# miuda-ai/lele

Hardware: AMD Instinct MI355X
Metric: STFT+mel GB/s (SenseVoice front-end: PCM -> log-mel -> LFR, algorithmic bytes); SenseVoiceSmall-shaped RTF in `sensevoice` (higher is better)
Workload: dtype f32

## Files before the change

### lele_amd/csrc/fe_core.h

```cpp
#pragma once
#include <stdint.h>

#if defined(__HIPCC__)
#define FE_HD __host__ __device__ __forceinline__
#else
#define FE_HD inline
#endif

namespace fe {

constexpr int kNfft = 512;
constexpr int kFrame = 400;
constexpr int kHop = 160;
constexpr int kBins = 257;
constexpr int kLanes = 16;
constexpr int kRegs = 32;
constexpr int kQ = 25;

FE_HD constexpr int rev4(int x) { return ((x & 1) << 3) | ((x & 2) << 1) | ((x & 4) >> 1) | ((x & 8) >> 3); }
FE_HD constexpr int rev5(int x) {
    return ((x & 1) << 4) | ((x & 2) << 2) | (x & 4) | ((x & 8) >> 2) | ((x & 16) >> 4);
}
FE_HD constexpr int tw_off(int s) { return (1 << (s - 1)) - 1; }

// ... 91 lines not shown
        if (rev5(r + 1) >= kQ) {
            s1[r] = x[r];
            s1[r + 1] = x[r];
        } else {
            s1[r] = fadd(x[r], x[r + 1]);
            s1[r + 1] = fsub(x[r], x[r + 1]);
        }
    }
    {
        const float wr = tw_re[tw_off(2) + 1], wi = tw_im[tw_off(2) + 1];
#pragma unroll
        for (int b = 0; b < kRegs; b += 4) {
            a[b] = cmk(fadd(s1[b], s1[b + 2]), 0.0f);
            a[b + 2] = cmk(fsub(s1[b], s1[b + 2]), 0.0f);
            const float tr = fmul(wr, s1[b + 3]);
            const float ti = fmul(wi, s1[b + 3]);
            a[b + 1] = cmk(fadd(s1[b + 1], tr), ti);
            a[b + 3] = cmk(fsub(s1[b + 1], tr), -ti);
        }
    }
#pragma unroll
    for (int b = 0; b < kRegs; b += 8) {
#pragma unroll
        for (int k = 0; k < 4; ++k) {
            const float wr = tw_re[tw_off(3) + k], wi = tw_im[tw_off(3) + k];
            if ((k & 1) == 0) {
                const float e = a[b + k].x, o = a[b + 4 + k].x;
                const float tr = fmul(wr, o);
                const float ti = fmul(wi, o);
                a[b + k] = cmk(fadd(e, tr), ti);
                a[b + 4 + k] = cmk(fsub(e, tr), -ti);
            } else {
                bfly_fma(make_tw(wr, wi), a[b + k], a[b + 4 + k]);
            }
        }
    }
#pragma unroll
    for (int s = 4; s <= 5; ++s) {
        const int half = 1 << (s - 1);
#pragma unroll
        for (int b = 0; b < kRegs; b += 2 * half) {
            {
                const cf e = a[b], o = a[b + half];
                a[b] = cadd(e, o);
                a[b + half] = csub(e, o);
            }
#pragma unroll
            for (int k = 1; k < half; ++k)
                bfly_fma(make_tw(tw_re[tw_off(s) + k], tw_im[tw_off(s) + k]), a[b + k], a[b + half + k]);
        }
    }
}

constexpr int kTwConstN = 31;
constexpr uint32_t kTwConstRe[kTwConstN] = {
    0x3f800000u, 0x3f800000u, 0xb33bbd2eu, 0x3f800000u, 0x3f3504f3u, 0xb33bbd2eu, 0xbf3504f3u, 0x3f800000u,
    0x3f6c835eu, 0x3f3504f3u, 0x3ec3ef15u, 0xb33bbd2eu, 0xbec3ef18u, 0xbf3504f3u, 0xbf6c8360u, 0x3f800000u,
    0x3f7b14beu, 0x3f6c835eu, 0x3f54db31u, 0x3f3504f3u, 0x3f0e39d9u, 0x3ec3ef15u, 0x3e47c5bcu, 0xb33bbd2eu,
    0xbe47c5c2u, 0xbec3ef18u, 0xbf0e39dcu, 0xbf3504f3u, 0xbf54db32u, 0xbf6c8360u, 0xbf7b14bfu};
constexpr uint32_t kTwConstIm[kTwConstN] = {
    0x80000000u, 0x80000000u, 0xbf800000u, 0x80000000u, 0xbf3504f3u, 0xbf800000u, 0xbf3504f3u, 0x80000000u,
    0xbec3ef16u, 0xbf3504f3u, 0xbf6c835eu, 0xbf800000u, 0xbf6c835eu, 0xbf3504f3u, 0xbec3ef10u, 0x80000000u,
    0xbe47c5c2u, 0xbec3ef16u, 0xbf0e39dau, 0xbf3504f3u, 0xbf54db32u, 0xbf6c835eu, 0xbf7b14bfu, 0xbf800000u,
    0xbf7b14beu, 0xbf6c835eu, 0xbf54db30u, 0xbf3504f3u, 0xbf0e39d9u, 0xbec3ef10u, 0xbe47c5c1u};
FE_HD bool tw_const_used(int i) {
    return i == tw_off(2) + 1 || (i >= tw_off(3) && i < tw_off(4)) || (i > tw_off(4) && i < tw_off(5)) ||
           (i > tw_off(5) && i < kTwConstN);
}
struct TwConst {
    bool im;
    FE_HD float operator[](int i) const { return __builtin_bit_cast(float, im ? kTwConstIm[i] : kTwConstRe[i]); }
};
inline bool tw_const_matches(const float* tw_re, const float* tw_im) {
    for (int i = 0; i < kTwConstN; ++i) {
        if (!tw_const_used(i)) continue;
        if (__builtin_bit_cast(uint32_t, tw_re[i]) != kTwConstRe[i] || __builtin_bit_cast(uint32_t, tw_im[i]) != kTwConstIm[i]) return false;
    }
    return true;
}

template <typename TWF>
FE_HD void phase_b(cf* b, int c, int rho, const TWF& twf, float* re256) {
#pragma unroll
    for (int s = 6; s <= 8; ++s) {
        const int hv = 1 << (s - 6);
#pragma unroll
        for (int k = 0; k < hv; ++k) {
            const cf w = twf(tw_off(s) + k * 32 + rho * 16 + c);
            const Tw tw = make_tw(w.x, w.y);
#pragma unroll
            for (int base = 0; base < 16; base += 2 * hv) bfly_fma(tw, b[base + k], b[base + hv + k]);
        }
    }
#pragma unroll
    for (int k = 0; k < 8; ++k) {
        const cf w = twf(tw_off(9) + k * 32 + rho * 16 + c);
        const cf t = tw_mul_fma(make_tw(w.x, w.y), b[8 + k]);
        if (k == 0) *re256 = fsub(b[0].x, t.x);
        b[k] = cadd(b[k], t);
    }
}


FE_HD float power(float re, float im) { return fadd(fmul(re, re), fmul(im, im)); }
FE_HD float power(cf z) {
    cf sq = cmulv(z, z);
// ... 12 lines not shown
```

### lele_amd/csrc/frontend.hip

```cpp
#include <type_traits>
#include "common.h"
#include "fe_core.h"

#include <math.h>

#include <algorithm>

using namespace lele;

namespace {

constexpr int kMaxMelRounds = 8;

struct FeDev {
    const float* tw_re;
    const float* tw_im;
    const float2* tw;
    const float* window;
    const float* melw;
    const float* melw_lds;
    const int* mel_start;
    const int* mel_step_off;
    int mel_rounds;
    int mel_steps;
    int n_mels;
    int lfr_m, lfr_n;
    int tile_dma;
};

struct GridBlock {
    __device__ __forceinline__ unsigned x() const { return blockIdx.x; }
    __device__ __forceinline__ unsigned y() const { return blockIdx.y; }
};
struct SegBlock {
    unsigned bx;
    __device__ __forceinline__ unsigned x() const { return bx; }
    __device__ __forceinline__ unsigned y() const { return 0u; }
};

struct FeSeg {
    int64_t start, len;
    int64_t num_frames, t_lfr;
    int64_t row0;
    int64_t block0;
};

constexpr int kSumRows = 66;
constexpr int kSumPitch = 164;

__global__ __launch_bounds__(64) void fe_frame_sum_kernel(const float* __restrict__ pcm, int64_t utt_stride,
                                                          int64_t pcm_len, int64_t num_frames,
                                                          float* __restrict__ mean_out, int aligned16) {
    __shared__ __attribute__((aligned(16))) float tile[kSumRows * kSumPitch];
    const int lane = threadIdx.x;
    const int64_t f0 = (int64_t)blockIdx.x * 64;
    const float* base = pcm + (int64_t)blockIdx.y * utt_stride;
    const int64_t s0 = f0 * fe::kHop;
    constexpr int kVecPerRow = fe::kHop / 4;
    constexpr int kVecs = kSumRows * kVecPerRow;
    constexpr int kIters = (kVecs + 63) / 64;
    constexpr int kBatch = 14;
    static_assert(kIters % kBatch == 0, "batching");
    for (int b0 = 0; b0 < kIters; b0 += kBatch) {
        float4 st[kBatch];
#pragma unroll
        for (int u = 0; u < kBatch; ++u) {
            const int idx = (b0 + u) * 64 + lane;
            int64_t s = s0 + 4 * (int64_t)idx;
            if (s + 3 >= pcm_len) s = aligned16 ? ((pcm_len - 4) & ~int64_t(3)) : (pcm_len - 4);
            if (s < 0) s = 0;
            const float* src = base + s;
            if (aligned16) {
                st[u] = *reinterpret_cast<const float4*>(src);
            } else {
                st[u] = make_float4(src[0], src[1], src[2], src[3]);
            }
        }
#pragma unroll
        for (int u = 0; u < kBatch; ++u) {
            const int idx = (b0 + u) * 64 + lane;
// ... 9 lines not shown
        }
    }
    __syncthreads();
    float sum = 0.0f;
#pragma unroll
    for (int seg = 0; seg < 3; ++seg) {
        const float* rowp = &tile[(lane + seg) * kSumPitch];
        const int nvec = seg < 2 ? kVecPerRow : (fe::kFrame - 2 * fe::kHop) / 4;
#pragma unroll 10
        for (int k = 0; k < nvec; ++k) {
            const float4 r = *reinterpret_cast<const float4*>(rowp + 4 * k);
            sum = sum + r.x;
            sum = sum + r.y;
            sum = sum + r.z;
            sum = sum + r.w;
        }
    }
    const int64_t f = f0 + lane;
    if (f < num_frames) mean_out[(int64_t)blockIdx.y * num_frames + f] = sum / (float)fe::kFrame;
}

constexpr int kFrameXchgFloats = 2 * 16 * fe::kXchgPitch;
constexpr int kWaveLdsFloats = 4 * kFrameXchgFloats;
constexpr int kPStride = 272;

struct TwLds {
    const float2* t;
    __device__ __forceinline__ float2 at(int i) const { return t[i]; }
};

__device__ __forceinline__ void fe_dma16(const void* gsrc, __attribute__((address_space(3))) char* lds_dst) {
    __builtin_amdgcn_global_load_lds((const __attribute__((address_space(1))) void*)gsrc, lds_dst, 16, 0, 0);
}

__device__ __forceinline__ const float* fe_const_table(const float* t, int pass) {
    auto c = (const __attribute__((address_space(4))) float*)t;
    asm("" : "+s"(c) : "s"(pass));
    return (const float*)c;
}

template <int MODE>
__device__ __forceinline__ float lane_rot_prev(float v, int p) {
    if (MODE == 1) {
        return __builtin_bit_cast(float,
                                  __builtin_amdgcn_update_dpp(0, __builtin_bit_cast(int, v), 0x121, 0xf, 0xf, true));
    } else {
        return __shfl(v, (p + 15) & 15, 16);
    }
}

constexpr int kStdMelLen[5] = {3, 4, 6, 10, 17};
constexpr int kStdMelOff[6] = {0, 3, 7, 13, 23, 40};

constexpr int kFeConstTw = 1, kFeLdsMel = 2, kFeLeanLds = 4;
typedef float fe_f2 __attribute__((ext_vector_type(2)));
typedef volatile __attribute__((address_space(3))) fe_f2* fe_lds_f2v;
__device__ __forceinline__ fe::cf fe_lds_read8(const float* p) {
    const fe_f2 t = *(fe_lds_f2v)p;
    return fe::cmk(t.x, t.y);
}
__device__ __forceinline__ void fe_lds_write8(float* p, fe::cf v) { *(fe_lds_f2v)p = (fe_f2){v.x, v.y}; }
constexpr int kMelLdsFloats = 768;
static_assert(fe::mel_lds_index(fe::kMelLdsWeights - 1, 15) < kMelLdsFloats && kStdMelOff[5] == fe::kMelLdsWeights, "the image holds the default bank");

template <int MODE, bool STDMEL, bool FUSED, int PASSES, bool LOWREG, int OPT, class Blk>
__device__ __forceinline__ void fe_main_body(const float* __restrict__ pcm, int64_t utt_stride,
                                             int64_t num_frames, int64_t t_lfr,
                                             const float* __restrict__ means, const FeDev& tb,
                                             float* __restrict__ out, float* __restrict__ logmel_out,
                                             int aligned16, float* s_melw, Blk bl) {
    constexpr int FR = 16 * PASSES;
    constexpr int kRows = FR + 2;
    constexpr int kXFloats = FUSED ? (kRows * kSumPitch > 4 * kWaveLdsFloats ? kRows * kSumPitch : 4 * kWaveLdsFloats)
                                   : 4 * kWaveLdsFloats;
    __shared__ float2 s_tw[LOWREG ? 480 : 512];
    __shared__ __attribute__((aligned(16))) float s_x[kXFloats];
    __shared__ float s_mean[64];
    __shared__ int s_mstart[16 * (STDMEL ? 5 : kMaxMelRounds)];
    __shared__ int s_moff[kMaxMelRounds + 1];
    constexpr int kTwBase = LOWREG ? 31 : 0;
    constexpr bool kConstTw = (OPT & kFeConstTw) != 0;
    constexpr bool kLdsMel = (OPT & kFeLdsMel) != 0;
    constexpr bool kLean = (OPT & kFeLeanLds) != 0;
    static_assert(!kLean || (kConstTw && kLdsMel), "the lean pass is a form of the constant-table kernel");
    static_assert(OPT == 0 || (STDMEL && FUSED && !LOWREG), "the constant / LDS table forms belong to the default bank's fused kernel");
    __shared__ __attribute__((aligned(16))) float s_melt[kLdsMel ? kMelLdsFloats : 4];
    static_assert(sizeof(s_tw) + sizeof(s_x) + sizeof(s_mean) + sizeof(s_mstart) + sizeof(s_moff) + sizeof(s_melt) <= 54613, "LDS of three workgroups fits a CU");

    const int lane = threadIdx.x & 63, wave = threadIdx.x >> 6;
    const int g = lane >> 4, p = lane & 15;
    constexpr int kVecPerRow = fe::kHop / 4;
    constexpr int kVecs = kRows * kVecPerRow;
    constexpr int kIters = (kVecs + 255) / 256;
    constexpr bool kTwDma = FUSED && !LOWREG;
    const bool tile_dma = FUSED && !LOWREG && aligned16 && tb.tile_dma;
    float4 st[FUSED ? kIters : 1];
    if constexpr (FUSED) {
        const float* run = pcm + (int64_t)bl.y() * utt_stride + (int64_t)bl.x() * FR * fe::kHop;
        const int64_t rem64 = utt_stride - (int64_t)bl.x() * FR * fe::kHop;
        const int rem = (int)(rem64 < (1 << 20) ? rem64 : (1 << 20));
        if (tile_dma) {
            constexpr int kSlotsPerRow = kSumPitch / 4;
            constexpr int kDma = (FR - 1 + 2) * kSlotsPerRow + (fe::kFrame - 2 * fe::kHop) / 4;
            constexpr int kDmaInstr = (kDma + 63) / 64;
            static_assert(kDmaInstr * 64 * 4 <= kXFloats, "the tile DMA stays inside s_x");
            auto* tile_lds = (__attribute__((address_space(3))) char*)s_x;
            static_assert(kSlotsPerRow == 41 && kDmaInstr * 64 * 1599 < (1 << 24), "i / 41 == (i * 1599) >> 16 for every slot");
            const unsigned last = 4u * (unsigned)rem - 16u;
            const int wave_s = __builtin_amdgcn_readfirstlane(wave);
#pragma unroll
            for (int u = 0; 4 * u < kDmaInstr; ++u) {
                const unsigned i = 256u * u + threadIdx.x;
                const unsigned ob = 16u * (i - ((i * 1599u) >> 16));
                if (4 * u + 3 < kDmaInstr || 4 * u + wave_s < kDmaInstr)
                    fe_dma16(reinterpret_cast<const char*>(run) + (ob < last ? ob : last), tile_lds + (4 * u + wave_s) * 1024);
            }
        }
        if (kTwDma && wave == 3) {
            auto* tw_lds = (__attribute__((address_space(3))) char*)s_tw;
#pragma unroll
            for (int k = 0; k < 4; ++k)
                fe_dma16(reinterpret_cast<const char*>(tb.tw) + 1024 * k + 16 * lane, tw_lds + 1024 * k);
        }
        if (kLdsMel && wave == 2) {
            auto* mel_lds = (__attribute__((address_space(3))) char*)s_melt;
#pragma unroll
            for (int k = 0; k < kMelLdsFloats / 256; ++k)
                fe_dma16(reinterpret_cast<const char*>(tb.melw_lds) + 1024 * k + 16 * lane, mel_lds + 1024 * k);
        }
        if (!tile_dma) {
#pragma unroll
            for (int u = 0; u < kIters; ++u) {
                const int idx = u * 256 + (int)threadIdx.x;
                int o = 4 * idx;
                if (o + 3 >= rem) o = aligned16 ? ((rem - 4) & ~3) : (rem - 4);
                const float* src = run + o;
                if (aligned16)
                    st[u] = *reinterpret_cast<const float4*>(src);
                else
                    st[u] = make_float4(src[0], src[1], src[2], src[3]);
            }
        }
    }
    if (!kTwDma)
        for (int i = threadIdx.x; i < 511 - kTwBase; i += 256) s_tw[i] = tb.tw[i + kTwBase];
    if (!STDMEL)
        for (int i = threadIdx.x; i < tb.mel_steps * 16; i += 256) s_melw[i] = tb.melw[i];
    if (threadIdx.x < tb.mel_rounds * 16) s_mstart[threadIdx.x] = tb.mel_start[threadIdx.x];
    if (threadIdx.x <= tb.mel_rounds) s_moff[threadIdx.x] = tb.mel_step_off[threadIdx.x];
    if (FUSED) {
        if (!tile_dma) {
#pragma unroll
            for (int u = 0; u < kIters; ++u) {
                const int idx = u * 256 + (int)threadIdx.x;
                if (idx < kVecs) {
                    const int row = idx / kVecPerRow, c = idx - row * kVecPerRow;
                    *reinterpret_cast<float4*>(&s_x[row * kSumPitch + 4 * c]) = st[u];
                }
            }
        }
        __builtin_amdgcn_s_waitcnt(0x0F70);
        __syncthreads();
    }
    const int h = fe::rev4(p);
    float* xw = s_x + wave * kWaveLdsFloats;
    float* xf = xw + g * kFrameXchgFloats;
    const float* base = pcm + (int64_t)bl.y() * utt_stride;
    const float* mean_u = means + (int64_t)bl.y() * num_frames;
    const int d_out = tb.n_mels * tb.lfr_m;
    float* out_u = out ? out + (int64_t)bl.y() * t_lfr * d_out : nullptr;
    float* lm_u = logmel_out ? logmel_out + (int64_t)bl.y() * num_frames * tb.n_mels : nullptr;

    float win[fe::kQ];
    if (!LOWREG) {
#pragma unroll
// ... 46 lines not shown
    const int f_first = (int)(bl.x() * FR) + wave * (4 * PASSES) + g;
    const int nfr = (int)num_frames, tl = (int)t_lfr;
    const int pad = (tb.lfr_m - 1) / 2;
    const unsigned blk_bytes = 4u * (unsigned)tb.n_mels, row_bytes = 4u * (unsigned)d_out;
    auto target_off = [&](int i, int b) { return (unsigned)i * row_bytes + (unsigned)b * blk_bytes + 4u * (unsigned)p; };
    int lfr_b = (f_first + pad) % tb.lfr_n, lfr_i = (f_first + pad) / tb.lfr_n;
    unsigned lfr_o = target_off(lfr_i, lfr_b);
    auto next_targets = [&]() {
        lfr_b += 4;
        if (tb.lfr_n >= 4) {
            const bool carry = lfr_b >= tb.lfr_n;
            lfr_b -= carry ? tb.lfr_n : 0;
            lfr_i += carry ? 1 : 0;
            lfr_o += carry ? 4u * blk_bytes + row_bytes - (unsigned)tb.lfr_n * blk_bytes : 4u * blk_bytes;
        } else {
            lfr_i += lfr_b / tb.lfr_n;
            lfr_b = lfr_b % tb.lfr_n;
            lfr_o = target_off(lfr_i, lfr_b);
        }
    };

    auto run_pass = [&](int pass, auto load_next_c) {
        constexpr bool load_next = decltype(load_next_c)::value;
        const int fi = f_first + pass * 4;
        const bool valid = fi < nfr;
        const float mean = FUSED ? s_mean[wave * (4 * PASSES) + pass * 4 + g] : mean_next;
        if (LOWREG) {
            int off = 0;
            asm volatile("" : "+v"(off));
#pragma unroll
            for (int q = 0; q < fe::kQ; ++q) win[q] = tb.window[p + 16 * q + off];
        }

        float v[fe::kQ];
        const float neg_mean = -mean;
#pragma unroll
        for (int q = 0; q < fe::kQ; ++q) v[q] = __builtin_fmaf(xr[q], 32768.0f, neg_mean);
        if (load_next) issue_loads(pass + 1);
        float xin[fe::kRegs];
#pragma unroll
        for (int r = 0; r < fe::kRegs; ++r) xin[r] = 0.0f;
        float k97;
        asm("v_mov_b32 %0, 0x3f7851ec" : "=v"(k97));
#pragma unroll
        for (int q = 0; q < fe::kQ; ++q) {
            const float send = (p == 15 && q > 0) ? v[q > 0 ? q - 1 : 0] : v[q];
            const float prev = lane_rot_prev<MODE>(send, p);
            float y = fe::fsub(v[q], fe::fmul(k97, prev));
            if (q == 0) y = (p == 0) ? v[0] : y;
            xin[fe::rev5(q)] = fe::fmul(y, win[q]);
        }

        fe::cf a[fe::kRegs];
        if constexpr (kConstTw)
            fe::phase_a_fast(xin, a, fe::TwConst{false}, fe::TwConst{true});
        else
            fe::phase_a_fast(xin, a, fe_const_table(tb.tw_re, pass), fe_const_table(tb.tw_im, pass));

        float pw[2][8];
        float p256 = 0.0f;
#pragma unroll
        for (int rho = 0; rho < 2; ++rho) {
            __builtin_amdgcn_wave_barrier();
#pragma unroll
            for (int cc = 0; cc < 16; ++cc) {
                const int slot = fe::xchg_slot(h, cc);
                if constexpr (kLean)
                    fe_lds_write8(xf + 2 * slot, a[rho * 16 + cc]);
                else
                    *reinterpret_cast<float2*>(xf + 2 * slot) = make_float2(a[rho * 16 + cc].x, a[rho * 16 + cc].y);
            }
            __builtin_amdgcn_wave_barrier();
            fe::cf bq[16];
#pragma unroll
            for (int vv = 0; vv < 16; ++vv) {
                if constexpr (kLean) {
                    bq[vv] = fe_lds_read8(xf + 2 * fe::xchg_slot(vv, p));
                } else {
                    const float2 t = *reinterpret_cast<const float2*>(xf + 2 * fe::xchg_slot(vv, p));
                    bq[vv] = fe::cmk(t.x, t.y);
                }
            }
            __builtin_amdgcn_wave_barrier();
            float re256 = 0.0f;
            fe::phase_b(bq, p, rho, [&](int i) { const float2 w = s_tw[i - kTwBase]; return fe::cmk(w.x, w.y); }, &re256);
            if (rho == 0) p256 = re256;
#pragma unroll
            for (int vv = 0; vv < 8; ++vv) {
                fe::cf z = bq[vv];
                if (vv == 0 && rho == 0) z = fe::cmk(z.x, (p == 0) ? 0.0f : z.y);
                pw[rho][vv] = fe::power(z);
            }
        }
        float* prow = xw + g * kPStride;
        __builtin_amdgcn_wave_barrier();
#pragma unroll
        for (int rho = 0; rho < 2; ++rho)
#pragma unroll
            for (int vv = 0; vv < 8; ++vv) prow[(2 * vv + rho) * 16 + p] = pw[rho][vv];
        if (p == 0) prow[256] = fe::power(p256, 0.0f);
        __builtin_amdgcn_wave_barrier();

        float vals[STDMEL ? 5 : kMaxMelRounds];
        float wl[kLdsMel ? fe::kMelLdsWeights : 1];
        if constexpr (kLdsMel) {
#pragma unroll
            for (int j = 0; j < fe::kMelLdsChunks; ++j) {
// ... 356 lines not shown
    const int per = n_mels / W;
    for (int v = lane; v < per * lfr_m; v += 64) {
        const int b = v / per, c = v - b * per;
        int64_t g = i * lfr_n + b - pad;
        g = g < 0 ? 0 : g;
        if (r.final) g = g > r.last_frame ? r.last_frame : g;
        LELE_DEV_ASSERT(g >= r.mel_base && g - r.mel_base < r.mel_carry + r.nf);
        const float* src = mel + (g - r.mel_base) * n_mels + W * c;
        float* d = dst + b * n_mels + W * c;
        if (VEC)
            __builtin_nontemporal_store(*reinterpret_cast<const fe_f4*>(src), reinterpret_cast<fe_f4*>(d));
        else
            __builtin_nontemporal_store(*src, d);
    }
}

__device__ __forceinline__ void fe_stream_move(float* region, int from, int count) {
    if (from == 0) return;
    for (int r0 = 0; r0 < count; r0 += 256 * kCompactRegs) {
        float v[kCompactRegs];
#pragma unroll
        for (int u = 0; u < kCompactRegs; ++u) {
            const int j = r0 + u * 256 + (int)threadIdx.x;
            v[u] = j < count ? region[from + j] : 0.0f;
        }
        __syncthreads();
#pragma unroll
        for (int u = 0; u < kCompactRegs; ++u) {
            const int j = r0 + u * 256 + (int)threadIdx.x;
            if (j < count) region[j] = v[u];
        }
    }
}
__global__ __launch_bounds__(256) void fe_stream_compact_kernel(const FeStreamRec* __restrict__ recs, float* pcm_state, int64_t pcm_pitch,
                                                                float* mel_state, int64_t mel_pitch, int n_mels) {
    const FeStreamRec r = recs[blockIdx.x];
    LELE_DEV_ASSERT(r.pcm_from + r.pcm_keep <= pcm_pitch && (int64_t)(r.mel_from + r.mel_keep) * n_mels <= mel_pitch);
    fe_stream_move(pcm_state + (int64_t)blockIdx.x * pcm_pitch, r.pcm_from, r.pcm_keep);
    fe_stream_move(mel_state + (int64_t)blockIdx.x * mel_pitch, r.mel_from * n_mels, r.mel_keep * n_mels);
}

}

struct LeleFrontend {
    LeleCtx* ctx = nullptr;
    LeleFeatureConfig cfg{};
    int64_t frame_len = 0, hop_len = 0, n_fft = 0;
    bool fast = false;
    bool std_mel = false;
    int dpp_mode = 0;
    bool fused = true;
    int opt = 0;
    bool lean = false;
    const float* g_window = nullptr;
    const int* g_mstart = nullptr;
    const int* g_moff = nullptr;
    const float* g_mw = nullptr;
    FeDev dev{};
    std::vector<void*> allocs;
    DevTables seg_tables;
    bool profiling = false;
    std::vector<hipEvent_t> events;
    size_t events_used = 0;
};

namespace {

static const float PI_F = 3.14159265358979323846264338327950288f;

void host_hann(int64_t size, std::vector<float>& w) {
    w.resize(size);
    if (size == 1) w[0] = 1.0f;
    for (int64_t n = 0; size > 1 && n < size; ++n) w[n] = 0.5f * (1.0f - cosf(2.0f * PI_F * (float)n / (float)(size - 1)));
}

void host_twiddles(int64_t n, std::vector<float>& re, std::vector<float>& im) {
    re.clear();
    im.clear();
    for (int64_t size = 2; size <= n; size *= 2) {
        int64_t half = size / 2, step = n / size;
        for (int64_t k = 0; k < half; ++k) {
            float angle = -2.0f * PI_F * (float)(k * step) / (float)n;
            re.push_back(cosf(angle));
            im.push_back(sinf(angle));
        }
    }
}

float hz_to_mel(float hz) { return 2595.0f * log10f(1.0f + hz / 700.0f); }
float mel_to_hz(float mel) { return 700.0f * (powf(10.0f, mel / 2595.0f) - 1.0f); }

void host_dense_mel(float sr, int64_t n_fft, int64_t n_mels, float f_min, float f_max, float* bank) {
    const int64_t n_freqs = n_fft / 2 + 1;
    const float mel_min = hz_to_mel(f_min), mel_max = hz_to_mel(f_max);
    const float mel_step = (mel_max - mel_min) / (float)(n_mels + 1);
    std::vector<float> hz(n_mels + 2), ff(n_freqs);
    for (int64_t i = 0; i < n_mels + 2; ++i) hz[i] = mel_to_hz(mel_min + (float)i * mel_step);
    for (int64_t i = 0; i < n_freqs; ++i) ff[i] = (float)i * sr / (float)n_fft;
    for (int64_t i = 0; i < n_mels; ++i) {
        const float fl = hz[i], fc = hz[i + 1], fr = hz[i + 2];
        for (int64_t j = 0; j < n_freqs; ++j) {
            const float f = ff[j];
            float val = 0.0f;
            if (f > fl && f < fc)
                val = (f - fl) / (fc - fl);
            else if (f >= fc && f < fr)
// ... 99 lines not shown
        return 0;
    }
    std::vector<float> win, twr, twi;
    host_hann(fe->frame_len, win);
    host_twiddles(fe->n_fft, twr, twi);
    for (int i : {0, 1, fe::tw_off(4), fe::tw_off(5)})
        LELE_REQUIRE(twr[i] == 1.0f && twi[i] == 0.0f, "frontend_create: unexpected twiddle table entry %d", i);
    std::vector<float2> tw(512, make_float2(0.f, 0.f));
    for (size_t i = 0; i < twr.size(); ++i) tw[i] = make_float2(twr[i], twi[i]);
    twr.resize(512, 0.0f);
    twi.resize(512, 0.0f);
    std::vector<int> mstart;
    std::vector<std::vector<float>> mw;
    host_sparse_mel((float)cfg->sample_rate, fe->n_fft, cfg->n_mels, 20.0f, mstart, mw);
    FeDev& d = fe->dev;
    d.n_mels = (int)cfg->n_mels;
    d.lfr_m = (int)cfg->lfr_m;
    d.lfr_n = (int)cfg->lfr_n;
    d.mel_rounds = (int)((cfg->n_mels + 15) / 16);
    std::vector<int> start_pad(d.mel_rounds * 16, 0);
    std::vector<float> melw;
    std::vector<int> step_off(d.mel_rounds + 1, 0);
    int off = 0;
    for (int rd = 0; rd < d.mel_rounds; ++rd) {
        size_t maxlen = 0;
        for (int pm = 0; pm < 16; ++pm) {
            int m = rd * 16 + pm;
            if (m < cfg->n_mels) {
                start_pad[m] = mstart[m];
                maxlen = std::max(maxlen, mw[m].size());
            }
        }
        step_off[rd] = off;
        for (size_t t = 0; t < maxlen; ++t)
            for (int pm = 0; pm < 16; ++pm) {
                int m = rd * 16 + pm;
                melw.push_back((m < cfg->n_mels && t < mw[m].size()) ? mw[m][t] : 0.0f);
            }
        off += (int)maxlen;
    }
    step_off[d.mel_rounds] = off;
    d.mel_steps = off;
    fe->std_mel = (d.mel_rounds == 5 && cfg->n_mels == 80);
    for (int rd = 0; fe->std_mel && rd < 5; ++rd) {
        if (step_off[rd] != kStdMelOff[rd] || step_off[rd + 1] != kStdMelOff[rd + 1]) fe->std_mel = false;
        for (int pm = 0; pm < 16; ++pm)
            if (start_pad[rd * 16 + pm] + kStdMelLen[rd] - 1 > 256) fe->std_mel = false;
    }
    if (lab_env("LELE_HIP_FE_GENERIC_MEL")) fe->std_mel = false;
    int rc = 0;
    rc |= upload(fe, twr, &d.tw_re);
    rc |= upload(fe, twi, &d.tw_im);
    rc |= upload(fe, tw, &d.tw);
    rc |= upload(fe, win, &d.window);
    rc |= upload(fe, melw, &d.melw);
    {
        std::vector<float> img(kMelLdsFloats, 0.0f);
        for (int sidx = 0; fe->std_mel && sidx < fe::kMelLdsWeights; ++sidx)
            for (int pm = 0; pm < 16; ++pm) img[fe::mel_lds_index(sidx, pm)] = melw[sidx * 16 + pm];
        rc |= upload(fe, img, &d.melw_lds);
    }
    rc |= upload(fe, start_pad, &d.mel_start);
    rc |= upload(fe, step_off, &d.mel_step_off);
    if (rc) {
        lele_hip_frontend_destroy(fe);
        return rc;
    }
    const char* env = lab_env("LELE_HIP_FE_DPP");
    fe->dpp_mode = env ? atoi(env) : 1;
    const char* envf = lab_env("LELE_HIP_FE_FUSED");
    fe->fused = envf ? atoi(envf) != 0 : true;
    const char* envd = getenv("LELE_HIP_FE_TILE_DMA");
    d.tile_dma = envd && *envd ? atoi(envd) != 0 : 1;
    const char* envc = getenv("LELE_HIP_FE_CONST_TW");
    const char* envl = getenv("LELE_HIP_FE_LDS_TABLES");
    bool const_tw = fe::tw_const_matches(twr.data(), twi.data());
    if (envc && !strcmp(envc, "mismatch")) {
        std::vector<float> other = twr;
        other[fe::tw_off(5) + 3] = nextafterf(other[fe::tw_off(5) + 3], 2.0f);
        const_tw = fe::tw_const_matches(other.data(), twi.data());
    } else if (envc && *envc && atoi(envc) == 0) {
        const_tw = false;
    }
    if (const_tw && fe->std_mel && fe->fused && fe->dpp_mode == 1)
        fe->opt = kFeConstTw | ((envl && *envl && atoi(envl) == 0) ? 0 : kFeLdsMel);
    const char* envn = getenv("LELE_HIP_FE_LEAN_LDS");
    fe->lean = fe->opt == (kFeConstTw | kFeLdsMel) && !(envn && *envn && atoi(envn) == 0);
    *out = fe;
    return 0;
}

int lele_hip_frontend_kernel_form(const LeleFrontend* fe) { return fe ? fe->opt : -1; }
int lele_hip_frontend_lean_lds(const LeleFrontend* fe) { return fe ? (int)fe->lean : -1; }

int lele_hip_frontend_destroy(LeleFrontend* fe) {
    if (!fe) return 0;
    (void)hipStreamSynchronize(fe->ctx->stream);
    for (void* p : fe->allocs) (void)hipFree(p);
    fe->seg_tables.release();
    for (hipEvent_t e : fe->events) (void)hipEventDestroy(e);
    delete fe;
    return 0;
}

int lele_hip_frontend_out_rows(const LeleFrontend* fe, int64_t pcm_len, int64_t* rows, int64_t* cols,
                               int64_t* num_frames) {
    LELE_REQUIRE(fe, "frontend_out_rows: fe is NULL");
    int64_t nf = 0, t = 0;
    if (pcm_len >= fe->frame_len) {
        nf = (pcm_len - fe->frame_len) / fe->hop_len + 1;
        t = (nf + fe->cfg.lfr_n - 1) / fe->cfg.lfr_n;
    }
    if (rows) *rows = t;
    if (cols) *cols = fe->cfg.n_mels * fe->cfg.lfr_m;
    if (num_frames) *num_frames = nf;
    return 0;
}

static int ilog2_i(int n) {
    int l = 0;
    while ((1 << (l + 1)) <= n) ++l;
    return l;
}
static int fe_generic(LeleFrontend* fe, const float* dpcm, int64_t batch, int64_t pcm_len, int64_t nf, int64_t t_lfr, int64_t cols,
                      float* outp, bool want_logmel, void* dmean) {
    LeleCtx* ctx = fe->ctx;
    const int64_t bins = fe->n_fft / 2 + 1, nm = fe->cfg.n_mels;
    if (fe->fused && fe->n_fft <= 4096 && fe->frame_len <= fe->n_fft && batch <= 65535) {
        const int n = (int)fe->n_fft;
        int fpb = n <= 512 ? 4 : n <= 1024 ? 2 : 1;
        if (const char* e = lab_env("LELE_HIP_FE_FPB")) fpb = std::max(1, atoi(e));
        const size_t padded = (size_t)fpb * n + (((size_t)fpb * n) >> 5) + 1;
        const size_t lds = (2 * padded + (size_t)fpb * bins + (size_t)(fpb - 1) * fe->hop_len + fe->frame_len + fpb) * 4;
        if (lds <= 96 * 1024) {
            ctx->set_route("fe.generic_fused");
            const float *twr = nullptr, *twi = nullptr;
            LELE_TRY(fft_twiddles(ctx, n, &twr, &twi));
            LELE_HIP_CHECK(ensure_dyn_lds(reinterpret_cast<const void*>(fe_generic_fused_kernel), (int)lds));
            const int64_t per_utt_lm = nf * nm * 4;
            const int64_t ubf = want_logmel ? batch : std::max<int64_t>(1, std::min<int64_t>(batch, (int64_t(1) << 28) / std::max<int64_t>(per_utt_lm, 1)));
            void* glm = nullptr;
            if (!want_logmel) LELE_TRY(ctx->arena_alloc((size_t)ubf * nf * nm * 4, &glm));
            for (int64_t u = 0; u < batch; u += ubf) {
                const int64_t nu = std::min<int64_t>(ubf, batch - u);
                const float* up = (const float*)dpcm + u * pcm_len;
                float* lm = want_logmel ? outp + u * nf * nm : (float*)glm;
// ... 63 lines not shown
    LELE_TRY(ctx->get_scratch((size_t)batch * nf * sizeof(float), &dmean));
    const size_t out_elems = want_logmel ? (size_t)batch * nf * fe->cfg.n_mels : (size_t)batch * t_lfr * cols;
    LELE_TRY(out->reserve(out_elems * sizeof(float)));
    if (!fe->fast) {
        LELE_TRY(fe_generic(fe, (const float*)dpcm, batch, pcm_len, nf, t_lfr, cols, (float*)out->data, want_logmel, dmean));
        if (want_logmel) {
            if (batch == 1) return set_shape(out_shape, out_rank, {nf, fe->cfg.n_mels});
            return set_shape(out_shape, out_rank, {batch, nf, fe->cfg.n_mels});
        }
        return 0;
    }
    LELE_REQUIRE((want_logmel ? nf * fe->cfg.n_mels : t_lfr * cols) < (int64_t(1) << 30),
                 "frontend: the features of one utterance (%lld frames) exceed 4 GiB", (long long)nf);
    const int aligned16 = ((uintptr_t)dpcm % 16 == 0) && (pcm_len % 4 == 0);
    ctx->set_route(fe->std_mel ? "fe.main_std" : "fe.main_table",
                   !fe->fused ? "fe.two_kernel" : (aligned16 && fe->dev.tile_dma) ? "fe.tile_dma" : "fe.tile_regs");
    constexpr int64_t kMaxGridY = 65535;
    hipEvent_t* ev = nullptr;
    if (fe->profiling) {
        if (fe->events_used + 3 > fe->events.size()) {
            for (int i = 0; i < 3; ++i) {
                hipEvent_t e;
                LELE_HIP_CHECK(hipEventCreate(&e));
                fe->events.push_back(e);
            }
        }
        ev = &fe->events[fe->events_used];
        fe->events_used += 3;
        LELE_HIP_CHECK(hipEventRecord(ev[0], ctx->stream));
    }
    for (int64_t c0 = 0; !fe->fused && c0 < batch; c0 += kMaxGridY) {
        const dim3 grid((unsigned)((nf + 63) / 64), (unsigned)std::min<int64_t>(kMaxGridY, batch - c0));
        hipLaunchKernelGGL(fe_frame_sum_kernel, grid, dim3(64), 0, ctx->stream, (const float*)dpcm + c0 * pcm_len, pcm_len, pcm_len, nf,
                           (float*)dmean + c0 * nf, aligned16);
    }
    if (ev) LELE_HIP_CHECK(hipEventRecord(ev[1], ctx->stream));
    const size_t mel_lds = fe->opt ? 0 : (size_t)fe->dev.mel_steps * 16 * sizeof(float);
#define FE_LAUNCH(MODE, STD, FUS, OPT)                                                                                               \
    hipLaunchKernelGGL((fe_main_kernel<MODE, STD, FUS, OPT>), grid, dim3(256), mel_lds, ctx->stream, cpcm, pcm_len, nf, t_lfr, cmean, fe->dev, \
                       o, lm, aligned16)
#define FE_LAUNCH2(MODE, STD) \
    do {                      \
        if (fe->fused)        \
            FE_LAUNCH(MODE, STD, true, 0); \
        else                  \
            FE_LAUNCH(MODE, STD, false, 0); \
    } while (0)
    for (int64_t c0 = 0; c0 < batch; c0 += kMaxGridY) {
        const dim3 grid((unsigned)((nf + 63) / 64), (unsigned)std::min<int64_t>(kMaxGridY, batch - c0));
        const float* cpcm = (const float*)dpcm + c0 * pcm_len;
        const float* cmean = (const float*)dmean + c0 * nf;
        float* o = want_logmel ? nullptr : (float*)out->data + c0 * t_lfr * cols;
        float* lm = want_logmel ? (float*)out->data + c0 * nf * fe->cfg.n_mels : nullptr;
        if (fe->lean) {
            FE_LAUNCH(1, true, true, kFeConstTw | kFeLdsMel | kFeLeanLds);
        } else if (fe->opt == (kFeConstTw | kFeLdsMel)) {
            FE_LAUNCH(1, true, true, kFeConstTw | kFeLdsMel);
        } else if (fe->opt == kFeConstTw) {
            FE_LAUNCH(1, true, true, kFeConstTw);
        } else if (fe->dpp_mode == 1) {
            if (fe->std_mel) FE_LAUNCH2(1, true); else FE_LAUNCH2(1, false);
        } else {
            if (fe->std_mel) FE_LAUNCH2(0, true); else FE_LAUNCH2(0, false);
        }
    }
#undef FE_LAUNCH2
#undef FE_LAUNCH
    LELE_HIP_CHECK(hipGetLastError());
    if (ev) LELE_HIP_CHECK(hipEventRecord(ev[2], ctx->stream));
    if (want_logmel) {
        if (batch == 1) return set_shape(out_shape, out_rank, {nf, fe->cfg.n_mels});
        return set_shape(out_shape, out_rank, {batch, nf, fe->cfg.n_mels});
    }
    return 0;
}

int lele_hip_frontend_compute(LeleFrontend* fe, const LeleTensor* pcm, LeleBuf* out, int64_t* out_shape,
                              int32_t* out_rank) {
    LELE_REQUIRE(fe && pcm && out, "frontend_compute: NULL argument");
    const int64_t n = numel(pcm);
    LELE_TRY(fe_run(fe, pcm, 1, n, out, false, out_shape, out_rank));
    if (out->bytes == 0) return 0;
    int64_t t = 0, cols = 0;
    lele_hip_frontend_out_rows(fe, n, &t, &cols, nullptr);
    return set_shape(out_shape, out_rank, {t, cols});
}

int lele_hip_frontend_compute_batch(LeleFrontend* fe, const LeleTensor* pcm, LeleBuf* out, int64_t* out_shape,
                                    int32_t* out_rank) {
    LELE_REQUIRE(fe && pcm && out, "frontend_compute_batch: NULL argument");
    LELE_REQUIRE(pcm->rank == 2, "frontend_compute_batch: pcm must be [batch, pcm_len]");
    const int64_t batch = pcm->shape[0], n = pcm->shape[1];
    LELE_TRY(fe_run(fe, pcm, batch, n, out, false, out_shape, out_rank));
    if (out->bytes == 0) return 0;
    int64_t t = 0, cols = 0;
    lele_hip_frontend_out_rows(fe, n, &t, &cols, nullptr);
    return set_shape(out_shape, out_rank, {batch, t, cols});
}

int lele_hip_frontend_logmel(LeleFrontend* fe, const LeleTensor* pcm, LeleBuf* out, int64_t* out_shape,
                             int32_t* out_rank) {
    LELE_REQUIRE(fe && pcm && out, "frontend_logmel: NULL argument");
    if (pcm->rank == 2) return fe_run(fe, pcm, pcm->shape[0], pcm->shape[1], out, true, out_shape, out_rank);
    return fe_run(fe, pcm, 1, numel(pcm), out, true, out_shape, out_rank);
}

struct SegLayout {
// ... 39 lines not shown
        row_offsets[i + 1] = row_offsets[i] + t;
        blocks += (nf + 63) / 64;
        max_nf = std::max(max_nf, nf);
    }
    const int64_t rows = row_offsets[count];
    fe->ctx->set_route(nullptr);
    if (rows == 0) {
        out->bytes = 0;
        if (out_rank) *out_rank = 0;
        return 0;
    }
    LELE_REQUIRE(blocks < (int64_t(1) << 31), "frontend_compute_segments: %lld blocks exceed the grid", (long long)blocks);
    LELE_REQUIRE(!fe->fast || (max_nf + fe->cfg.lfr_n - 1) / fe->cfg.lfr_n * cols < (int64_t(1) << 30),
                 "frontend_compute_segments: the features of one segment (%lld frames) exceed 4 GiB", (long long)max_nf);
    LeleCtx* ctx = fe->ctx;
    LELE_HIP_CHECK(hipSetDevice(ctx->device));
    LELE_TRY(ctx->arena_reset());
    const void* dpcm = nullptr;
    LELE_TRY(ctx->dev_ptr(pcm, &dpcm));
    LELE_TRY(out->reserve((size_t)rows * cols * sizeof(float)));
    float* o = (float*)out->data;
    if (!fe->fast) {
        void* dmean = nullptr;
        LELE_TRY(ctx->get_scratch((size_t)max_nf * sizeof(float), &dmean));
        const size_t mark = ctx->arena_used;
        for (int64_t i = 0; i < count; ++i) {
            int64_t t = 0, nf = 0;
            lele_hip_frontend_out_rows(fe, lengths[i], &t, nullptr, &nf);
            if (nf == 0) continue;
            LELE_TRY(fe_generic(fe, (const float*)dpcm + starts[i], 1, lengths[i], nf, t, cols, o + row_offsets[i] * cols, false, dmean));
            ctx->arena_used = mark;
        }
        return set_shape(out_shape, out_rank, {rows, cols});
    }
    std::string key((size_t)count * 16, '\0');
    memcpy(&key[0], starts, (size_t)count * 8);
    memcpy(&key[(size_t)count * 8], lengths, (size_t)count * 8);
    const SegLayout lay{fe, starts, lengths, count, row_offsets};
    const void* table = nullptr;
    LELE_TRY(fe->seg_tables.get(ctx, std::move(key), build_seg_table, &lay, &table));
    int64_t nseg = 0;
    for (int64_t i = 0; i < count; ++i) nseg += lengths[i] >= fe->frame_len;
    const FeSeg* dsegs = (const FeSeg*)table;
    const int* dblk = (const int*)(dsegs + nseg);
    const size_t mel_lds = fe->opt ? 0 : (size_t)fe->dev.mel_steps * 16 * sizeof(float);
    int64_t n_dma = 0;
    for (int64_t i = 0; i < count; ++i)
        if (lengths[i] >= fe->frame_len)
            n_dma += (((uintptr_t)((const float*)dpcm + starts[i]) & 15) == 0) && (lengths[i] % 4 == 0) && fe->dev.tile_dma;
    ctx->set_route(fe->std_mel ? "fe.seg_std" : "fe.seg_table", n_dma == nseg ? "fe.tile_dma" : n_dma == 0 ? "fe.tile_regs" : "fe.tile_mixed");
#define FE_SEG_LAUNCH(MODE, STD, ...)                                                                                            \
    hipLaunchKernelGGL((fe_seg_main_kernel<MODE, STD, ##__VA_ARGS__>), dim3((unsigned)blocks), dim3(256), mel_lds, ctx->stream, (const float*)dpcm, \
                       dsegs, dblk, fe->dev, o)
    if (fe->lean) {
        FE_SEG_LAUNCH(1, true, kFeConstTw | kFeLdsMel | kFeLeanLds);
    } else if (fe->opt == (kFeConstTw | kFeLdsMel)) {
        FE_SEG_LAUNCH(1, true, kFeConstTw | kFeLdsMel);
    } else if (fe->opt == kFeConstTw) {
        FE_SEG_LAUNCH(1, true, kFeConstTw);
    } else if (fe->dpp_mode == 1) {
        if (fe->std_mel) FE_SEG_LAUNCH(1, true); else FE_SEG_LAUNCH(1, false);
    } else {
        if (fe->std_mel) FE_SEG_LAUNCH(0, true); else FE_SEG_LAUNCH(0, false);
    }
#undef FE_SEG_LAUNCH
    LELE_HIP_CHECK(hipGetLastError());
    return set_shape(out_shape, out_rank, {rows, cols});
}

}

namespace {
struct FeStreamDims {
    int64_t frame_len, hop, m, n, pad;
    int64_t frames(int64_t len) const { return len < frame_len ? 0 : (len - frame_len) / hop + 1; }
    int64_t rows(int64_t t) const { return t - 1 >= m - 1 - pad ? (t - 1 - (m - 1 - pad)) / n + 1 : 0; }
    int64_t rows_final(int64_t t) const { return (t + n - 1) / n; }
    int64_t pcm_carry(int64_t len, int64_t t) const { return t == 0 ? len : std::max<int64_t>(0, len - t * hop); }
    int64_t mel_carry(int64_t t, int64_t e) const { return std::max<int64_t>(0, t - std::max<int64_t>(0, e * n - pad)); }
};
int fe_stream_dims(const LeleFeatureConfig* cfg, FeStreamDims* d) {
    LELE_REQUIRE(cfg->sample_rate > 0 && cfg->n_mels > 0 && cfg->lfr_m > 0 && cfg->lfr_n > 0, "frontend_stream: invalid FeatureConfig");
    d->frame_len = (int64_t)((float)cfg->sample_rate * cfg->frame_length_ms / 1000.0f);
    d->hop = (int64_t)((float)cfg->sample_rate * cfg->frame_shift_ms / 1000.0f);
    d->m = cfg->lfr_m;
    d->n = cfg->lfr_n;
    d->pad = (cfg->lfr_m - 1) / 2;
    LELE_REQUIRE(d->frame_len >= 1 && d->hop >= 1, "frontend_stream: frame_len=%lld hop_len=%lld", (long long)d->frame_len, (long long)d->hop);
    return 0;
}
}

struct LeleFrontendStream {
    LeleFrontend* fe = nullptr;
    hipStream_t stream = nullptr;
    FeStreamDims dims{};
    int64_t streams = 0, max_chunk = 0;
    int64_t max_new_frames = 0;
    float* pcm_state = nullptr;
    float* mel_state = nullptr;
    int64_t pcm_pitch = 0, mel_pitch = 0;
    std::vector<int64_t> samples, frames, rows;
};

extern "C" {

int lele_hip_frontend_stream_rows(const LeleFeatureConfig* cfg, int64_t samples_before, int64_t chunk_len, int32_t final, int64_t* rows,
// ... 137 lines not shown
        }
        blk.insert(blk.end(), (size_t)((r.nf + 63) / 64), (int)i);
        eblk.insert(eblk.end(), (size_t)((r.rows + kEmitRows - 1) / kEmitRows), (int)i);
        row_offsets[i + 1] = row_offsets[i] + r.rows;
        max_chunk = std::max<int64_t>(max_chunk, lengths[i]);
        max_nf = std::max<int64_t>(max_nf, r.nf);
        n_live += r.nf > 0;
        n_dma += r.nf > 0 && len % 4 == 0 && fe->dev.tile_dma;
        nl[(size_t)i] = fin ? 0 : L2;
        nt[(size_t)i] = fin ? 0 : T2;
        ne[(size_t)i] = fin ? 0 : E2;
    }
    const int64_t total_rows = row_offsets[count];
    const int64_t pieces = (max_chunk + kAppendPiece - 1) / kAppendPiece;
    LELE_REQUIRE(count * pieces < (int64_t(1) << 31) && blk.size() < (size_t(1) << 31) && eblk.size() < (size_t(1) << 31),
                 "frontend_stream_push: %lld streams of up to %lld samples exceed the grid", (long long)count, (long long)max_chunk);
    LELE_HIP_CHECK(hipSetDevice(ctx->device));
    ctx->set_route(nullptr);
    LELE_TRY(ctx->arena_reset());
    const void* dpcm = nullptr;
    LELE_TRY(ctx->dev_ptr(pcm, &dpcm));
    const size_t rec_bytes = recs.size() * sizeof(FeStreamRec), blk_bytes = blk.size() * sizeof(int), eblk_bytes = eblk.size() * sizeof(int);
    std::vector<char> blob(rec_bytes + blk_bytes + eblk_bytes);
    memcpy(blob.data(), recs.data(), rec_bytes);
    if (blk_bytes) memcpy(blob.data() + rec_bytes, blk.data(), blk_bytes);
    if (eblk_bytes) memcpy(blob.data() + rec_bytes + blk_bytes, eblk.data(), eblk_bytes);
    void* dtab = nullptr;
    LELE_TRY(ctx->arena_alloc(blob.size(), &dtab));
    void* dmean = nullptr;
    if (!fe->fast && max_nf) LELE_TRY(ctx->get_scratch((size_t)max_nf * sizeof(float), &dmean));
    if (total_rows) LELE_TRY(out->reserve((size_t)total_rows * cols * sizeof(float)));
    LELE_HIP_CHECK(hipMemcpyAsync(dtab, blob.data(), blob.size(), hipMemcpyHostToDevice, ctx->stream));
    const FeStreamRec* drecs = (const FeStreamRec*)dtab;
    const int* dblk = (const int*)((const char*)dtab + rec_bytes);
    const int* deblk = (const int*)((const char*)dtab + rec_bytes + blk_bytes);
    if (pieces)
        hipLaunchKernelGGL(fe_stream_append_kernel, dim3((unsigned)(count * pieces)), dim3(64), 0, ctx->stream, (const float*)dpcm, drecs, (int)pieces,
                           st->pcm_state, st->pcm_pitch);
    if (n_live && !fe->fast) {
        const size_t mark = ctx->arena_used;
        for (int64_t i = 0; i < count; ++i) {
            const FeStreamRec& r = recs[(size_t)i];
            if (r.nf == 0) continue;
            LELE_TRY(fe_generic(fe, st->pcm_state + i * st->pcm_pitch, 1, (int64_t)r.carry + r.chunk, r.nf, 0, cols,
                                st->mel_state + i * st->mel_pitch + (int64_t)r.mel_carry * nm, true, dmean));
            ctx->arena_used = mark;
        }
    } else if (n_live) {
        ctx->set_route(fe->std_mel ? "fe.seg_std" : "fe.seg_table", n_dma == n_live ? "fe.tile_dma" : n_dma == 0 ? "fe.tile_regs" : "fe.tile_mixed");
        const size_t mel_lds = fe->opt ? 0 : (size_t)fe->dev.mel_steps * 16 * sizeof(float);
#define FE_STREAM_LAUNCH(MODE, STD, ...)                                                                                           \
    hipLaunchKernelGGL((fe_stream_main_kernel<MODE, STD, ##__VA_ARGS__>), dim3((unsigned)blk.size()), dim3(256), mel_lds, ctx->stream,              \
                       (const float*)st->pcm_state, st->pcm_pitch, drecs, dblk, fe->dev, st->mel_state, st->mel_pitch)
        if (fe->lean) {
            FE_STREAM_LAUNCH(1, true, kFeConstTw | kFeLdsMel | kFeLeanLds);
        } else if (fe->opt == (kFeConstTw | kFeLdsMel)) {
            FE_STREAM_LAUNCH(1, true, kFeConstTw | kFeLdsMel);
        } else if (fe->opt == kFeConstTw) {
            FE_STREAM_LAUNCH(1, true, kFeConstTw);
        } else if (fe->dpp_mode == 1) {
            if (fe->std_mel) FE_STREAM_LAUNCH(1, true); else FE_STREAM_LAUNCH(1, false);
        } else {
            if (fe->std_mel) FE_STREAM_LAUNCH(0, true); else FE_STREAM_LAUNCH(0, false);
        }
#undef FE_STREAM_LAUNCH
    }
    if (total_rows) {
        if (nm % 4 == 0)
            hipLaunchKernelGGL(fe_stream_emit_kernel<true>, dim3((unsigned)eblk.size()), dim3(256), 0, ctx->stream, (const float*)st->mel_state,
                               st->mel_pitch, drecs, deblk, (int)nm, (int)d.m, (int)d.n, (float*)out->data);
        else
            hipLaunchKernelGGL(fe_stream_emit_kernel<false>, dim3((unsigned)eblk.size()), dim3(256), 0, ctx->stream, (const float*)st->mel_state,
                               st->mel_pitch, drecs, deblk, (int)nm, (int)d.m, (int)d.n, (float*)out->data);
    }
    if (moves)
        hipLaunchKernelGGL(fe_stream_compact_kernel, dim3((unsigned)count), dim3(256), 0, ctx->stream, drecs, st->pcm_state, st->pcm_pitch,
                           st->mel_state, st->mel_pitch, (int)nm);
    LELE_HIP_CHECK(hipGetLastError());
    st->samples.swap(nl);
    st->frames.swap(nt);
    st->rows.swap(ne);
    if (total_rows == 0) {
        out->bytes = 0;
        if (out_rank) *out_rank = 0;
        return 0;
    }
    return set_shape(out_shape, out_rank, {total_rows, cols});
}

int lele_hip_frontend_set_profiling(LeleFrontend* fe, int on) {
    LELE_REQUIRE(fe, "frontend_set_profiling: fe is NULL");
    fe->profiling = on != 0;
    fe->events_used = 0;
    return 0;
}

int lele_hip_frontend_profile_read(LeleFrontend* fe, float* sum_kernel_ms, float* main_kernel_ms, int64_t* runs) {
    LELE_REQUIRE(fe, "frontend_profile_read: fe is NULL");
    LELE_HIP_CHECK(hipStreamSynchronize(fe->ctx->stream));
    double a = 0, b = 0;
    const size_t n = fe->events_used / 3;
    for (size_t i = 0; i < n; ++i) {
        float m0 = 0, m1 = 0;
        LELE_HIP_CHECK(hipEventElapsedTime(&m0, fe->events[3 * i], fe->events[3 * i + 1]));
        LELE_HIP_CHECK(hipEventElapsedTime(&m1, fe->events[3 * i + 1], fe->events[3 * i + 2]));
        a += m0;
        b += m1;
// ... 10 lines not shown
```

Before: 1997.

## Add conjugate-symmetric phase A that tracks real and conjugated FFT registers

Adds a phase_a_conj variant of the first radix stages. It keeps purely real registers as scalars and stores some complex registers in conjugated ("primed") form, so stages skip imaginary arithmetic and sign negations. A conjugated twiddle table is built on the host and DMA'd into LDS for the later phase, so it matches the primed layout. The variant is enabled by default under the lean LDS path, with an environment switch to turn it off. It risks subtle sign errors, which a constexpr static_assert over the class bookkeeping is meant to guard against.

```diff
diff --git a/lele_amd/csrc/fe_core.h b/lele_amd/csrc/fe_core.h
--- a/lele_amd/csrc/fe_core.h
+++ b/lele_amd/csrc/fe_core.h
@@ -167,6 +167,98 @@
     }
 }
 
+FE_HD constexpr bool primed(int r) { return r == 8 || ((0x2636 >> (r & 15)) & 1) != 0; }
+enum : int { kClsReal = 0, kClsNormal = 1, kClsPrimed = 2 };
+FE_HD constexpr int conj_class(int s, int r) {
+    if (s <= 1) return kClsReal;
+    const int half = 1 << (s - 1), k = r & (half - 1);
+    if (k == 0) return kClsReal;
+    if (k == half / 2 && conj_class(s - 1, r) == kClsReal) return (r & half) ? kClsNormal : kClsPrimed;
+    return conj_class(s - 1, r);
+}
+FE_HD constexpr bool conj_classes_hold() {
+    for (int s = 2; s <= 5; ++s) {
+        const int half = 1 << (s - 1);
+        for (int b = 0; b < kRegs; b += 2 * half)
+            for (int k = 0; k < half; ++k) {
+                const int ce = conj_class(s - 1, b + k), co = conj_class(s - 1, b + half + k);
+                if (ce != co) return false;
+                if ((k == 0 || k == half / 2) != (ce == kClsReal)) return false;
+                if (ce != kClsReal && (ce == kClsPrimed) != primed(b + k)) return false;
+                if (ce != kClsReal && (co == kClsPrimed) != primed(b + half + k)) return false;
+            }
+    }
+    for (int r = 0; r < kRegs; ++r) {
+        if ((conj_class(5, r) == kClsReal) != (r == 0 || r == 16)) return false;
+        if ((conj_class(5, r) == kClsPrimed) != primed(r)) return false;
+    }
+    return true;
+}
+static_assert(conj_classes_hold(), "phase_a_conj never pairs a primed register with a normal one, and ends in primed(r)");
+
+template <typename TW>
+FE_HD void phase_a_conj(const float* x, cf* a, const TW& tw_re, const TW& tw_im) {
+    float s1[kRegs];
+#pragma unroll
+    for (int r = 0; r < kRegs; r += 2) {
+        if (rev5(r + 1) >= kQ) {
+            s1[r] = x[r];
+            s1[r + 1] = x[r];
+        } else {
+            s1[r] = fadd(x[r], x[r + 1]);
+            s1[r + 1] = fsub(x[r], x[r + 1]);
+        }
+    }
+    float re[kRegs];
+    {
+        const float wr = tw_re[tw_off(2) + 1], nwi = -tw_im[tw_off(2) + 1];
+#pragma unroll
+        for (int b = 0; b < kRegs; b += 4) {
+            re[b] = fadd(s1[b], s1[b + 2]);
+            re[b + 2] = fsub(s1[b], s1[b + 2]);
+            const float tr = fmul(wr, s1[b + 3]);
+            const float nti = fmul(nwi, s1[b + 3]);
+            a[b + 1] = cmk(fadd(s1[b + 1], tr), nti);
+            a[b + 3] = cmk(fsub(s1[b + 1], tr), nti);
+        }
+    }
+#pragma unroll
+    for (int s = 3; s <= 5; ++s) {
+        const int half = 1 << (s - 1);
+#pragma unroll
+        for (int b = 0; b < kRegs; b += 2 * half) {
+#pragma unroll
+            for (int k = 0; k < half; ++k) {
+                const int i = b + k, j = b + half + k;
+                if (k == 0) {
+                    const float e = re[i], o = re[j];
+                    re[i] = fadd(e, o);
+                    re[j] = fsub(e, o);
+                } else if (k == half / 2) {
+                    const float wr = tw_re[tw_off(s) + k], nwi = -tw_im[tw_off(s) + k];
+                    const float e = re[i], o = re[j];
+                    const float tr = fmul(wr, o);
+                    const float nti = fmul(nwi, o);
+                    a[i] = cmk(fadd(e, tr), nti);
+                    a[j] = cmk(fsub(e, tr), nti);
+                } else {
+                    const float wr = tw_re[tw_off(s) + k], wi = tw_im[tw_off(s) + k];
+                    bfly_fma(make_tw(wr, primed(i) ? -wi : wi), a[i], a[j]);
+                }
+            }
+        }
+    }
+    a[0] = cmk(re[0], 0.0f);
+    a[16] = cmk(re[16], 0.0f);
+}
+
+inline void tw_conj_image(const float* tw_re, const float* tw_im, int n, float* out ) {
+    for (int i = 0; i < n; ++i) {
+        out[2 * i] = tw_re[i];
+        out[2 * i + 1] = (i >= tw_off(6) && primed((i + 1) & 31)) ? -tw_im[i] : tw_im[i];
+    }
+}
+
 constexpr int kTwConstN = 31;
 constexpr uint32_t kTwConstRe[kTwConstN] = {
     0x3f800000u, 0x3f800000u, 0xb33bbd2eu, 0x3f800000u, 0x3f3504f3u, 0xb33bbd2eu, 0xbf3504f3u, 0x3f800000u,
diff --git a/lele_amd/csrc/frontend.hip b/lele_amd/csrc/frontend.hip
--- a/lele_amd/csrc/frontend.hip
+++ b/lele_amd/csrc/frontend.hip
@@ -26,6 +26,7 @@
     int n_mels;
     int lfr_m, lfr_n;
     int tile_dma;
+    const float2* tw_conj;
 };
 
 struct GridBlock {
@@ -141,7 +142,7 @@
 constexpr int kStdMelLen[5] = {3, 4, 6, 10, 17};
 constexpr int kStdMelOff[6] = {0, 3, 7, 13, 23, 40};
 
-constexpr int kFeConstTw = 1, kFeLdsMel = 2, kFeLeanLds = 4;
+constexpr int kFeConstTw = 1, kFeLdsMel = 2, kFeLeanLds = 4, kFeConjA = 8;
 typedef float fe_f2 __attribute__((ext_vector_type(2)));
 typedef volatile __attribute__((address_space(3))) fe_f2* fe_lds_f2v;
 __device__ __forceinline__ fe::cf fe_lds_read8(const float* p) {
@@ -171,7 +172,9 @@
     constexpr bool kConstTw = (OPT & kFeConstTw) != 0;
     constexpr bool kLdsMel = (OPT & kFeLdsMel) != 0;
     constexpr bool kLean = (OPT & kFeLeanLds) != 0;
+    constexpr bool kConj = (OPT & kFeConjA) != 0;
     static_assert(!kLean || (kConstTw && kLdsMel), "the lean pass is a form of the constant-table kernel");
+    static_assert(!kConj || kLean, "the conjugate phase A is a form of the lean pass");
     static_assert(OPT == 0 || (STDMEL && FUSED && !LOWREG), "the constant / LDS table forms belong to the default bank's fused kernel");
     __shared__ __attribute__((aligned(16))) float s_melt[kLdsMel ? kMelLdsFloats : 4];
     static_assert(sizeof(s_tw) + sizeof(s_x) + sizeof(s_mean) + sizeof(s_mstart) + sizeof(s_moff) + sizeof(s_melt) <= 54613, "LDS of three workgroups fits a CU");
@@ -209,7 +212,7 @@
             auto* tw_lds = (__attribute__((address_space(3))) char*)s_tw;
 #pragma unroll
             for (int k = 0; k < 4; ++k)
-                fe_dma16(reinterpret_cast<const char*>(tb.tw) + 1024 * k + 16 * lane, tw_lds + 1024 * k);
+                fe_dma16(reinterpret_cast<const char*>(kConj ? tb.tw_conj : tb.tw) + 1024 * k + 16 * lane, tw_lds + 1024 * k);
         }
         if (kLdsMel && wave == 2) {
             auto* mel_lds = (__attribute__((address_space(3))) char*)s_melt;
@@ -362,7 +365,9 @@
         }
 
         fe::cf a[fe::kRegs];
-        if constexpr (kConstTw)
+        if constexpr (kConj)
+            fe::phase_a_conj(xin, a, fe::TwConst{false}, fe::TwConst{true});
+        else if constexpr (kConstTw)
             fe::phase_a_fast(xin, a, fe::TwConst{false}, fe::TwConst{true});
         else
             fe::phase_a_fast(xin, a, fe_const_table(tb.tw_re, pass), fe_const_table(tb.tw_im, pass));
@@ -825,6 +830,7 @@
     bool fused = true;
     int opt = 0;
     bool lean = false;
+    bool conj = false;
     const float* g_window = nullptr;
     const int* g_mstart = nullptr;
     const int* g_moff = nullptr;
@@ -1030,6 +1036,11 @@
     rc |= upload(fe, twr, &d.tw_re);
     rc |= upload(fe, twi, &d.tw_im);
     rc |= upload(fe, tw, &d.tw);
+    {
+        std::vector<float2> twc(512, make_float2(0.f, 0.f));
+        fe::tw_conj_image(twr.data(), twi.data(), 511, reinterpret_cast<float*>(twc.data()));
+        rc |= upload(fe, twc, &d.tw_conj);
+    }
     rc |= upload(fe, win, &d.window);
     rc |= upload(fe, melw, &d.melw);
     {
@@ -1064,12 +1075,15 @@
         fe->opt = kFeConstTw | ((envl && *envl && atoi(envl) == 0) ? 0 : kFeLdsMel);
     const char* envn = getenv("LELE_HIP_FE_LEAN_LDS");
     fe->lean = fe->opt == (kFeConstTw | kFeLdsMel) && !(envn && *envn && atoi(envn) == 0);
+    const char* enva = getenv("LELE_HIP_FE_CONJ_A");
+    fe->conj = fe->lean && !(enva && *enva && atoi(enva) == 0);
     *out = fe;
     return 0;
 }
 
 int lele_hip_frontend_kernel_form(const LeleFrontend* fe) { return fe ? fe->opt : -1; }
 int lele_hip_frontend_lean_lds(const LeleFrontend* fe) { return fe ? (int)fe->lean : -1; }
+int lele_hip_frontend_conj_a(const LeleFrontend* fe) { return fe ? (int)fe->conj : -1; }
 
 int lele_hip_frontend_destroy(LeleFrontend* fe) {
     if (!fe) return 0;
@@ -1239,7 +1253,9 @@
         const float* cmean = (const float*)dmean + c0 * nf;
         float* o = want_logmel ? nullptr : (float*)out->data + c0 * t_lfr * cols;
         float* lm = want_logmel ? (float*)out->data + c0 * nf * fe->cfg.n_mels : nullptr;
-        if (fe->lean) {
+        if (fe->conj) {
+            FE_LAUNCH(1, true, true, kFeConstTw | kFeLdsMel | kFeLeanLds | kFeConjA);
+        } else if (fe->lean) {
             FE_LAUNCH(1, true, true, kFeConstTw | kFeLdsMel | kFeLeanLds);
         } else if (fe->opt == (kFeConstTw | kFeLdsMel)) {
             FE_LAUNCH(1, true, true, kFeConstTw | kFeLdsMel);
@@ -1385,7 +1401,9 @@
 #define FE_SEG_LAUNCH(MODE, STD, ...)                                                                                            \
     hipLaunchKernelGGL((fe_seg_main_kernel<MODE, STD, ##__VA_ARGS__>), dim3((unsigned)blocks), dim3(256), mel_lds, ctx->stream, (const float*)dpcm, \
                        dsegs, dblk, fe->dev, o)
-    if (fe->lean) {
+    if (fe->conj) {
+        FE_SEG_LAUNCH(1, true, kFeConstTw | kFeLdsMel | kFeLeanLds | kFeConjA);
+    } else if (fe->lean) {
         FE_SEG_LAUNCH(1, true, kFeConstTw | kFeLdsMel | kFeLeanLds);
     } else if (fe->opt == (kFeConstTw | kFeLdsMel)) {
         FE_SEG_LAUNCH(1, true, kFeConstTw | kFeLdsMel);
@@ -1629,7 +1647,9 @@
 #define FE_STREAM_LAUNCH(MODE, STD, ...)                                                                                           \
     hipLaunchKernelGGL((fe_stream_main_kernel<MODE, STD, ##__VA_ARGS__>), dim3((unsigned)blk.size()), dim3(256), mel_lds, ctx->stream,              \
                        (const float*)st->pcm_state, st->pcm_pitch, drecs, dblk, fe->dev, st->mel_state, st->mel_pitch)
-        if (fe->lean) {
+        if (fe->conj) {
+            FE_STREAM_LAUNCH(1, true, kFeConstTw | kFeLdsMel | kFeLeanLds | kFeConjA);
+        } else if (fe->lean) {
             FE_STREAM_LAUNCH(1, true, kFeConstTw | kFeLdsMel | kFeLeanLds);
         } else if (fe->opt == (kFeConstTw | kFeLdsMel)) {
             FE_STREAM_LAUNCH(1, true, kFeConstTw | kFeLdsMel);
```

Result: faster. 2020 (median of 6 runs) (+1.2%).
